# HybridRobotics/ilqr-iterative-tasks

Hardware: AMD Instinct MI355X
Metric: batched iLQR iterations/s (n=6,m=2,N=20) (higher is better)
Workload: dtype f64

## Files before the change

ilqr_iterative_tasks_amd/csrc/i2lqr_column_launch.hpp:

```cpp
#pragma once
#include <hip/hip_runtime.h>

#include "i2lqr_column_plan.hpp"
#include "i2lqr_devcfg.hpp"
#include "i2lqr_group.h"
#include "i2lqr_handle.hpp"
#include "i2lqr_host.hpp"
#include "i2lqr_kernels.h"
#include "i2lqr_wave_opt.h"

namespace i2lqr {

inline thread_local i2lqr_handle::Epilogue* t_epi = nullptr;

inline int64_t registered_ws(const i2lqr_handle* h) { return h->ws ? h->ws_bytes : -1; }
inline ColumnChoice column_kernel(const i2lqr_handle* h, int64_t B, bool early_exit) {
  return column_kernel(h->geo, h->fit, h->col, h->model.form(), registered_ws(h), B, early_exit);
}

inline int wave_lds_check(const i2lqr_handle* h, bool chained) {
  const size_t need = wave_lds_need(h->fit, h->model, chained);
  if (need <= h->geo.max_dyn_lds) return I2LQR_OK;
  const WaveForm f = h->model.form(chained);
  const int n_obs = h->model.records();
  char with[64];
  if (f == WAVE_OBS)
    snprintf(with, sizeof(with), "\"obstacles\" = %d", n_obs);
  else
    snprintf(with, sizeof(with), "%s and %d obstacle record%s",
             chained ? "\"wave_chain\"" : wave_phrase(f), n_obs, n_obs > 1 ? "s" : "");
  return fail(I2LQR_ERR_UNSUPPORTED, "horizon %d with %s needs %zu B of LDS per wavefront (> %zu KiB)",
              h->cfg.N, with, need, h->geo.max_dyn_lds / 1024);
}

template <class T, class Sys> struct Launch {
  static constexpr int n = Sys::n, m = Sys::m, LANES = 64;
  static constexpr bool kBicycle = m == 2 && n + m <= 8;
  using Cfg = DevCfg<T, n, m>;

  static unsigned grid(int64_t B) { return (unsigned)B; }

  static int prepare(i2lqr_handle* h) {
    h->lanes = LANES;
    h->fit.lds_wave = (size_t)Layout<Sys>(h->cfg.N).total * sizeof(T);
    h->fit.lds_wave_fstep = kWaveHasFstep<Sys> ? wave_fstep_lds_bytes<T, Sys>(h->cfg.N) : 0;
    const size_t lds = h->fit.lds_wave;
    if (lds > h->geo.max_dyn_lds)
      return fail(I2LQR_ERR_UNSUPPORTED, "horizon %d needs %zu B of LDS per wavefront (> %zu KiB)",
                  h->cfg.N, lds, h->geo.max_dyn_lds / 1024);
    if (lds > h->geo.default_dyn_lds)
      for (const void* kernel :
           {(const void*)k_iterate<T, Sys, LANES, false>, (const void*)k_iterate<T, Sys, LANES, true>,
            (const void*)k_backward<T, Sys, LANES, false>, (const void*)k_backward<T, Sys, LANES, true>,
            (const void*)k_forward<T, Sys, LANES, false>, (const void*)k_forward<T, Sys, LANES, true>,
            (const void*)k_rollout<T, Sys, LANES, false>, (const void*)k_rollout<T, Sys, LANES, true>})
        HIP_TRY(hipFuncSetAttribute(kernel, hipFuncAttributeMaxDynamicSharedMemorySize, (int)lds));
    return I2LQR_OK;
  }

  static int iterate(i2lqr_handle* h, const SolveIO& io, hipStream_t s) {
    const int64_t B = io.B;
    IterArgs<T> a = iter_args<T>(io);
    a.chains = h->col.opt_group_chains != 0;
#ifdef I2LQR_STAMPS
    a.dbg = (unsigned long long*)h->ws;
#endif
    const ColumnChoice choice = column_kernel(h, B, io.early_exit != 0);
    const ColumnKernel fk = choice.kernel;
    if (t_epi && (fk == K_GROUP || fk == K_GROUP16 || fk == K_GROUP_WS)) {
      a.qfun = t_epi->qfun;
      a.outer_iter = t_epi->outer_iter;
      a.max_relax_iter = t_epi->max_relax_iter;
      a.cost_it = (T*)t_epi->cost_it;
      if (t_epi->best_idx) {
        a.pick_part = (MinPair<T>*)t_epi->part;
        a.pick_ticket = h->ticket + h->ticket_next.fetch_add(1, std::memory_order_relaxed) %
                                        i2lqr_handle::kTickets;
        a.best_idx = t_epi->best_idx;
        a.best_cost = (T*)t_epi->best_cost;
      }
      t_epi->fused = true;
    }
#ifdef I2LQR_STAMPS
    constexpr bool stamps = true;
#else
    constexpr bool stamps = false;
#endif
    switch (fk) {
      case K_INVALID:
        return fail(I2LQR_ERR_UNSUPPORTED, "%s", choice.why);
      case K_SPEC:
      case K_SPEC16:
        if constexpr (kBicycle) {
          const int lanes = fk == K_SPEC16 ? 16 : 8;
          HIP_TRY(group_spec_iterate<T>(h->cfg, a, s, lanes,
                                        spec_wavefronts(h->geo, h->fit, lanes, B, false)));
          return I2LQR_OK;
        }
        break;
      case K_GROUP:
        if constexpr (kBicycle) {
          HIP_TRY(group_iterate<T>(h->cfg, a, s, stamps ? 1 : group8_wavefronts(h->geo, B)));
          return I2LQR_OK;
        }
        break;
      case K_GROUP16:
        if constexpr (kBicycle) {
          const int wavefronts =
              stamps ? 1 : group16_wavefronts(h->geo, B, h->col.opt_group_overlap != 0);
          HIP_TRY(group16_iterate<T>(h->cfg, a, s, wavefronts, !stamps && group16_fixed(h->fit, h->col)));
          return I2LQR_OK;
        }
        break;
      case K_GROUP_WS:
        if constexpr (kBicycle) {
          HIP_TRY(group_iterate_ws<T>(h->cfg, a, h->ws, s));
          return I2LQR_OK;
        }
        break;
      case K_QUAD:
        if constexpr (n + m == 16) {
          HIP_TRY(quad_iterate<T>(h->cfg, a, h->ws, s));
          return I2LQR_OK;
        }
        break;
      case K_WAVE_OPT:
        if (int rc = wave_lds_check(h, false)) return rc;
        HIP_TRY(wave_opt_launch<T>(h->cfg, a, h->model, false, h->fit.lds_wave, s));
        return I2LQR_OK;
      case K_WAVE:
        break;
    }
    const Cfg c = make_dev_cfg<T, n, m>(h->cfg);
    if constexpr (kWaveHasFstep<Sys>) {
      if (wave_fstep(h->geo, h->fit, h->col, B)) {
        with_weights(c.flags, [&](auto W) {
          hipLaunchKernelGGL((k_iterate<T, Sys, LANES, W, true>), dim3(grid(B)), dim3(64),
                             h->fit.lds_wave_fstep, s, c, a);
        });
        HIP_TRY(hipGetLastError());
        return I2LQR_OK;
      }
    }
    with_weights(c.flags, [&](auto W) {
      hipLaunchKernelGGL((k_iterate<T, Sys, LANES, W>), dim3(grid(B)), dim3(64), h->fit.lds_wave, s, c, a);
    });
    HIP_TRY(hipGetLastError());
    return I2LQR_OK;
  }
  static int names_pair(const i2lqr_handle*, int64_t, int) { return 0; }
  static int names_model(const i2lqr_handle*) { return 0; }
  static int solve_chained(i2lqr_handle* h, const SolveIO& io, int k, hipStream_t s) {
    const ChainPlan plan = chain_plan(h->geo, h->fit, h->col, h->model.form(), registered_ws(h), io.B);
    if (plan.kind == ChainPlan::REFUSED) return fail(I2LQR_ERR_UNSUPPORTED, "%s", plan.why);
    IterArgs<T> a = iter_args<T>(io);
    a.chain_len = k;
    a.chains = h->col.opt_group_chains != 0;
    if (plan.kind == ChainPlan::WAVE) {
      if (int rc = wave_lds_check(h, true)) return rc;
      HIP_TRY(wave_opt_launch<T>(h->cfg, a, h->model, true, h->fit.lds_wave, s));
    } else if constexpr (kBicycle) {
      HIP_TRY(group_spec_chain<T>(h->cfg, a, s));
    }
    return I2LQR_OK;
  }
  static int rollout(i2lqr_handle* h, int64_t B, void* X, void* U, const void* x_term, void* cost,
                     hipStream_t s) {
    const Cfg c = make_dev_cfg<T, n, m>(h->cfg);
    with_weights(c.flags, [&](auto W) {
      hipLaunchKernelGGL((k_rollout<T, Sys, LANES, W>), dim3(grid(B)), dim3(64), h->fit.lds_wave, s, c,
                         B, (T*)X, (T*)U, (const T*)x_term, (T*)cost);
    });
    HIP_TRY(hipGetLastError());
    return I2LQR_OK;
  }
  static int backward(i2lqr_handle* h, int64_t B, const void* X, const void* U, const void* x_term,
                      const void* lamb, const void* obs, void* K, void* k, hipStream_t s) {
    const Cfg c = make_dev_cfg<T, n, m>(h->cfg);
    with_weights(c.flags, [&](auto W) {
      hipLaunchKernelGGL((k_backward<T, Sys, LANES, W>), dim3(grid(B)), dim3(64), h->fit.lds_wave, s, c,
                         B, (const T*)X, (const T*)U, (const T*)x_term, (const T*)lamb,
                         (const T*)obs, (T*)K, (T*)k);
    });
    HIP_TRY(hipGetLastError());
    return I2LQR_OK;
  }
  static int forward(i2lqr_handle* h, int64_t B, const void* X, const void* U, const void* x_term,
                     const void* K, const void* k, void* Xn, void* Un, void* cost_new,
                     hipStream_t s) {
    const Cfg c = make_dev_cfg<T, n, m>(h->cfg);
    with_weights(c.flags, [&](auto W) {
      hipLaunchKernelGGL((k_forward<T, Sys, LANES, W>), dim3(grid(B)), dim3(64), h->fit.lds_wave, s, c,
                         B, (const T*)X, (const T*)U, (const T*)x_term, (const T*)K, (const T*)k,
                         (T*)Xn, (T*)Un, (T*)cost_new);
    });
    HIP_TRY(hipGetLastError());
    return I2LQR_OK;
  }
};

}
```

ilqr_iterative_tasks_amd/csrc/i2lqr_group.hpp:

```cpp
#pragma once
#include <hip/hip_runtime.h>
#include <stdint.h>

#include "i2lqr_systems.hpp"
#include "i2lqr_wave.hpp"

namespace i2lqr {

constexpr int kGroup = 8;
constexpr int kGroupsPerWave = 64 / kGroup;

template <class Sys> struct GroupPattern {
  static constexpr int n = Sys::n, m = Sys::m, W = n + m, NV = Sys::NVAR;
  static constexpr int dt_row(int b) {
    for (int i = 2; i < n; i++)
      if (i != b && Sys::pat(i, b) == 2) return i;
    return -1;
  }
  static constexpr bool column_ok(int b) {
    int extra = 0;
    for (int i = 0; i < n; i++) {
      const int code = Sys::pat(i, b);
      if (i < 2) {
        if (code == 2) return false;
        if (i == b && code != 1) return false;
        continue;
      }
      if (i == b) {
        if (code != 1) return false;
      } else if (code == 2) {
        extra++;
      } else if (code != 0) {
        return false;
      }
    }
    return extra <= 1;
  }
  static constexpr bool ok() {
    if (W > kGroup || n + 1 > kGroup || n < 2) return false;
    for (int b = 0; b < W; b++)
      if (!column_ok(b)) return false;
    return true;
  }
};

#ifndef I2LQR_GROUP_UNROLL
#define I2LQR_GROUP_UNROLL 4
#endif
template <class Sys, int G = kGroup> struct GLayout {
  static constexpr int n = Sys::n, m = Sys::m, W = n + m, NV = Sys::NVAR, NT = Sys::NTRIG;
  static constexpr int PW = 64 / G;
  static constexpr int KW = (n + 1 + 1) & ~1;
  static constexpr int R_JV = 0, R_ZERO = NV, R_ONE = NV + 1, R_LU = NV + 2, R_LUU = NV + 2 + m,
                       R_OB = NV + 2 + 2 * m, RW = (NV + 2 + 2 * m + 5 + 1) & ~1;
  int N;
  static constexpr int kT1Stride = 80;
  int XU0, XU1, Kk, R, TR0, TR1, total;
  __host__ __device__ explicit GLayout(int N_, bool ws = false) : N(N_) {
    int o = 0;
    XU0 = o; o += W * (N + 1); o = (o + 3) & ~3;
    XU1 = o; o += W * (N + 1); o = (o + 3) & ~3;
    Kk = o; o += ws ? m * KW : m * KW * N; o = (o + 3) & ~3;
    R = o; o += ws ? 0 : RW * (N + 1);
    TR0 = o; o += NT * (N + 1); o = (o + 3) & ~3;
    TR1 = o; o += NT * (N + 1); o = (o + 3) & ~3;
    o = (o + 3) & ~3;
    if (((o / 4) & 1) == 0) o += 4;
    total = o;
  }
  __host__ __device__ int t1_base() const { return PW * total; }
  __host__ __device__ int qt_base() const { return t1_base() + (G == kGroup ? PW * kT1Stride : 0); }
  __host__ __device__ int ctl_base() const { return (qt_base() + n * n + 3) & ~3; }
  __host__ __device__ int wave_words() const { return ctl_base() + 16; }
  __host__ __device__ int ws_rec() const { return 0; }
  __host__ __device__ int ws_gain() const { return RW * (N + 1); }
  __host__ __device__ int ws_words() const { return (RW * (N + 1) + m * KW * N + 15) & ~15; }
};


template <int L> __device__ __forceinline__ void bcast_fmac1(double& a, double s, double c) {
  asm("v_fmac_f64_dpp %0, %1, %2 row_newbcast:%3 row_mask:0xf bank_mask:0xf" : "+v"(a) : "v"(s), "v"(c), "n"(L));
}
template <int L> __device__ __forceinline__ void bcast_fmac1(float& a, float s, float c) {
  asm("v_fmac_f32_dpp %0, %1, %2 row_newbcast:%3 row_mask:0xf bank_mask:0xf" : "+v"(a) : "v"(s), "v"(c), "n"(L));
}
template <int L, class T, int R>
__device__ __forceinline__ void bcast_fmac(T (&a)[R], const T (&s)[R], T c) {
#pragma unroll
  for (int r = 0; r < R; r++) bcast_fmac1<L>(a[r], s[r], c);
}
template <int L> __device__ __forceinline__ double bcast_mov(double v) {
  long long x = __builtin_bit_cast(long long, v);
  x = __builtin_amdgcn_mov_dpp(x, 0x150 + L, 0xf, 0xf, false);
  return __builtin_bit_cast(double, x);
}
template <int L> __device__ __forceinline__ float bcast_mov(float v) {
  int x = __builtin_bit_cast(int, v);
  x = __builtin_amdgcn_mov_dpp(x, 0x150 + L, 0xf, 0xf, false);
  return __builtin_bit_cast(float, x);
}
template <class T, int R> __device__ __forceinline__ void dpp_ready(T (&v)[R]) {
  if constexpr (R == 8)
    asm("s_nop 1" : "+v"(v[0]), "+v"(v[1]), "+v"(v[2]), "+v"(v[3]), "+v"(v[4]), "+v"(v[5]), "+v"(v[6]), "+v"(v[7]));
  else if constexpr (R == 6)
    asm("s_nop 1" : "+v"(v[0]), "+v"(v[1]), "+v"(v[2]), "+v"(v[3]), "+v"(v[4]), "+v"(v[5]));
  else static_assert(R == 6 || R == 8, "dpp_ready: n + m of the bicycles");
}

template <class T, class Sys, bool WS = false, int G = kGroup, int NH = 0> struct GroupWorker {
  static constexpr int n = Sys::n, m = Sys::m, W = n + m, NV = Sys::NVAR, NT = Sys::NTRIG;
  static constexpr int NA = n + 1;
  using Cfg = DevCfg<T, n, m>;
  using GL = GLayout<Sys, G>;
  static_assert(G == kGroup || G == 16, "eight lanes per problem, or one 16-lane DPP row");
  static_assert(G == kGroup || !WS, "the workspace form is built for eight lanes per problem");
  static_assert(NH == 0 || (G == 16 && !WS), "the fixed-horizon form is the sixteen-lane LDS form");
  static __host__ __device__ constexpr int horizon(int cfg_N) { return NH > 0 ? NH : cfg_N; }
  using GP = GroupPattern<Sys>;
  static_assert(GP::ok(), "plant does not have the column structure this kernel is written for");
  const Cfg& c;
  const GL L;
  const Slice<T> S;
  const T* const Qt;
  const int g;
  const int N;
  __device__ __forceinline__ int loop_N() const {
    if constexpr (NH > 0) return c.N;
    else return N;
  }
  int oR, oKk;
  T* T1c;
  int rho;
  T* Wp = nullptr;

  int off_c0, off_c1;
  int off_l0, off_l1;
  int off_lu[m];
  T own, cdt;
  int rsrc;
#ifdef I2LQR_STAMPS
  mutable unsigned long long st_acc[8] = {0, 0, 0, 0, 0, 0, 0, 0}, st_t0 = 0, st_t1 = 0;
#endif

  __device__ GroupWorker(const Cfg& c_, T* smem, int lane)
      : GroupWorker(c_, smem + (lane / G) * GL(horizon(c_.N), WS).total,
                    smem + GL(horizon(c_.N), WS).qt_base(), lane % G,
                    GL(horizon(c_.N), WS).total) {
    const int p = lane / G;
    if constexpr (G == kGroup) T1c = smem + L.t1_base() + p * GL::kT1Stride;
    rho = (p >> 1) & 1;
  }
  __device__ __forceinline__ T* rec(int t) const {
    if constexpr (WS) return Wp + L.ws_rec() + t * GL::RW;
    else return S + oR + t * GL::RW;
  }
  __device__ __forceinline__ T* gain(int t) const {
    if constexpr (WS) return Wp + L.ws_gain() + t * (m * GL::KW);
    else return S + oKk + t * (m * GL::KW);
  }
  __device__ __forceinline__ T* gain_x(int t) const {
    if constexpr (WS) return S + oKk;
    else return S + oKk + t * (m * GL::KW);
  }
  __device__ __forceinline__ void ws_publish() const {
    if constexpr (WS) {
      __builtin_amdgcn_fence(__ATOMIC_RELEASE, "workgroup");
      __builtin_amdgcn_s_waitcnt(0);
      wave_sync();
      __builtin_amdgcn_fence(__ATOMIC_ACQUIRE, "workgroup");
    }
  }
  __device__ __forceinline__ int t1_word(int col, int row) const {
    return (row >> 1) * (2 * kGroup) + ((col + rho) & (kGroup - 1)) * 2 + (row & 1);
  }

  __device__ GroupWorker(const Cfg& c_, T* slice, const T* qt, int g_, int slice_words)
      : c(c_), L(horizon(c_.N), WS), S(make_slice(slice, slice_words, c_.trap, TAG_GROUP_LDS)),
        Qt(qt), g(g_), N(horizon(c_.N)) {
    oR = L.R; oKk = L.Kk;
    T1c = nullptr;
    rho = 0;
    off_c0 = GL::R_ZERO; off_c1 = GL::R_ZERO; off_l0 = GL::R_ZERO; off_l1 = GL::R_ZERO;
#pragma unroll
    for (int a = 0; a < m; a++) off_lu[a] = GL::R_ZERO;
    own = T(0); cdt = T(0); rsrc = 0;
    static_for_i<0, W>([&](auto b_) {
      constexpr int b = decltype(b_)::value;
      if (g == b && b < n) {
        constexpr int c0 = Sys::pat(0, b), c1 = Sys::pat(1, b);
        off_c0 = c0 == 0 ? GL::R_ZERO : (c0 == 1 ? GL::R_ONE : GL::R_JV + (c0 - 3));
        off_c1 = c1 == 0 ? GL::R_ZERO : (c1 == 1 ? GL::R_ONE : GL::R_JV + (c1 - 3));
        own = (b >= 2) ? T(1) : T(0);
        constexpr int r = GP::dt_row(b);
        cdt = r >= 0 ? c.dt : T(0);
        rsrc = r >= 0 ? r : 0;
        if (b < 2) {
          off_l0 = GL::R_OB + 2 + b;
          off_l1 = GL::R_OB + 3 + b;
        }
      }
    });
    if (g == n) {
      own = T(1);
      off_l0 = GL::R_OB + 0;
      off_l1 = GL::R_OB + 1;
#pragma unroll
      for (int a = 0; a < m; a++) off_lu[a] = GL::R_LU + a;
    }
    if constexpr (G == 16) {
      own = T(1);
      if (g == 0) off_c0 = GL::R_ZERO;
      if (g == 1) off_c1 = GL::R_ZERO;
    }
  }

  __device__ __forceinline__ T terminal_cost(const T (&x)[n], const T (&xT)[n]) const {
    T d[n];
#pragma unroll
    for (int i = 0; i < n; i++) d[i] = x[i] - xT[i];
    T acc = T(0);
#pragma unroll
    for (int j = 0; j < n; j++) {
      T col = T(0);
#pragma unroll
      for (int i = 0; i < n; i++) col += d[i] * Qt[i * n + j];
      acc += col * d[j];
    }
    return acc;
  }

  template <int i, int a> __device__ __forceinline__ void f_acc(T& acc, bool& first, T v,
                                                                const T (&jv)[NV]) const {
    constexpr int code = Sys::pat(i, a);
    if constexpr (code == 0) {
      return;
    } else if constexpr (code == 1) {
      acc = first ? v : acc + v;
      first = false;
    } else {
      const T f = code == 2 ? c.dt : jv[code >= 3 ? code - 3 : 0];
      acc = first ? f * v : t_fma(f, v, acc);
      first = false;
    }
  }

  __device__ __forceinline__ T rollout(int XUo, int TRo, const T (&xT)[n], bool chains) const {
    if constexpr (G == 16 && Sys::kTrigFreeTail) {
      if (__builtin_expect(chains, 1)) return rollout_row(XUo, TRo, xT);
    }
    T x[n], u[m], xn[n], tr[NT];
#pragma unroll
    for (int i = 0; i < n; i++) x[i] = S[XUo + i];
    const int N = loop_N();
    for (int t = 0; t < N; t++) {
#pragma unroll
      for (int a = 0; a < m; a++) u[a] = clip(S[XUo + t * W + n + a], -c.u_max[a], c.u_max[a]);
#pragma unroll
      for (int a = 0; a < m; a++) S[XUo + t * W + n + a] = u[a];
      Sys::trig(x, tr);
#pragma unroll
      for (int q = 0; q < NT; q++) S[TRo + t * NT + q] = tr[q];
      Sys::step_tr(c, x, u, tr, xn);
#pragma unroll
      for (int i = 0; i < n; i++) S[XUo + (t + 1) * W + i] = xn[i];
#pragma unroll
      for (int i = 0; i < n; i++) x[i] = xn[i];
    }
    Sys::trig(x, tr);
#pragma unroll
    for (int q = 0; q < NT; q++) S[TRo + N * NT + q] = tr[q];
    const T cost = terminal_cost(x, xT);
    wave_sync();
    return cost;
  }

  __device__ __forceinline__ T rollout_row(int XUo, int TRo, const T (&xT)[n]) const {
    static_assert(G == 16 && Sys::kTrigFreeTail, "see Sys::kTrigFreeTail");
    const int N = loop_N();
    for (int t = g; t < N; t += G) {
      T u[m];
#pragma unroll
      for (int a = 0; a < m; a++) u[a] = clip(S[XUo + t * W + n + a], -c.u_max[a], c.u_max[a]);
#pragma unroll
      for (int a = 0; a < m; a++) S[XUo + t * W + n + a] = u[a];
    }
    wave_sync();
    T x[n], u[m], xn[n], tr[NT];
#pragma unroll
    for (int i = 0; i < n; i++) x[i] = S[XUo + i];
#pragma unroll
    for (int q = 0; q < NT; q++) tr[q] = T(0);
    for (int t = 0; t < N; t++) {
#pragma unroll
      for (int a = 0; a < m; a++) u[a] = S[XUo + t * W + n + a];
      Sys::step_tr(c, x, u, tr, xn);
#pragma unroll
      for (int i = 2; i < n; i++) S[XUo + (t + 1) * W + i] = xn[i];
#pragma unroll
      for (int i = 2; i < n; i++) x[i] = xn[i];
    }
    const int rounds = (N + G) / G;
    for (int r = 0; r < rounds; r++) {
      const int t0 = g + r * G;
      const int t = t0 < N ? t0 : N;
      T xe[n];
      xe[0] = T(0); xe[1] = T(0);
#pragma unroll
      for (int i = 2; i < n; i++) xe[i] = S[XUo + t * W + i];
      Sys::trig(xe, tr);
#pragma unroll
      for (int q = 0; q < NT; q++) S[TRo + t * NT + q] = tr[q];
    }
    wave_sync();
    T un[m], trn[NT];
#pragma unroll
    for (int i = 0; i < n; i++) x[i] = S[XUo + i];
#pragma unroll
    for (int a = 0; a < m; a++) u[a] = S[XUo + n + a];
#pragma unroll
    for (int q = 0; q < NT; q++) tr[q] = S[TRo + q];
    for (int t = 0; t < N; t++) {
#pragma unroll
      for (int a = 0; a < m; a++) un[a] = S[XUo + (t + 1) * W + n + a];
#pragma unroll
      for (int q = 0; q < NT; q++) trn[q] = S[TRo + (t + 1) * NT + q];
      Sys::step_tr(c, x, u, tr, xn);
#pragma unroll
      for (int i = 0; i < n; i++) S[XUo + (t + 1) * W + i] = xn[i];
#pragma unroll
      for (int i = 0; i < n; i++) x[i] = xn[i];
#pragma unroll
      for (int a = 0; a < m; a++) u[a] = un[a];
#pragma unroll
      for (int q = 0; q < NT; q++) tr[q] = trn[q];
    }
    const T cost = terminal_cost(x, xT);
    wave_sync();
    return cost;
  }

  __device__ __forceinline__ void prep(int XUo, int TRo, const T (&ob)[6], T pa, T pb, int first,
                                       int stride, bool chains) const {
    if (__builtin_expect(chains, 1)) {
      if (sizeof(T) == 8 && __builtin_expect(c.fast_barrier, 1))
        prep_chains<true>(XUo, TRo, ob, pa, pb, first, stride);
      else
        prep_chains<false>(XUo, TRo, ob, pa, pb, first, stride);
    } else {
      prep_serial(XUo, TRo, ob, pa, pb, first, stride);
    }
    wave_sync();
    ws_publish();
  }

  template <bool FASTB>
  __device__ __forceinline__ void prep_chains(int XUo, int TRo, const T (&ob)[6], T pa, T pb,
                                              int first, int stride) const {
    static_assert(m == 2, "two inputs");
    const bool has_ob = ob[5] >= T(0);
    const int opt = has_ob ? (int)ob[5] : 0;
    const T spd_y = opt == 1 ? ob[4] : T(0), spd_x = opt == 2 ? ob[4] : T(0);
    const int rounds = (N + stride) / stride;
    for (int r = 0; r < rounds; r++) {
      const int t0 = first + r * stride;
      const int t = t0 < N ? t0 : N;
      const int ts = t0 < N ? t0 : N - 1;
      T* Rs = rec(ts);
      T* R = rec(t);
      if constexpr (FASTB) asm volatile("; record, short input barrier" ::: "memory");
      else asm volatile("; record, general input barrier" ::: "memory");
      T xe[n], tr[NT], u[m], jv[NV];
#pragma unroll
      for (int i = 0; i < n; i++) xe[i] = S[XUo + (ts + 1) * W + i];
#pragma unroll
      for (int a = 0; a < m; a++) u[a] = S[XUo + ts * W + n + a];
#pragma unroll
      for (int q = 0; q < NT; q++) tr[q] = S[TRo + (ts + 1) * NT + q];
      const T px = S[XUo + t * W + 0], py = S[XUo + t * W + 1];
      const T dz = opt == 2 ? px - (ob[0] - T(t) * spd_x) : px - ob[0];
      const T dy = opt == 1 ? py - (ob[1] + T(t) * spd_y) : py - ob[1];
      const T h = T(1) + c.safety_margin - (dz * pa * dz + dy * pb * dy);
      const T hd0 = T(-2) * pa * dz, hd1 = T(-2) * pb * dy;
      T e, e_hi[m], e_lo[m];
      if constexpr (FASTB) {
        const double xa[3] = {(double)(c.obs_q2 * h), (double)(c.ctrl_q2 * (u[0] - c.u_max[0])),
                              (double)(c.ctrl_q2 * (u[1] - c.u_max[1]))};
        double ea[3], rc[2];
        t_exp_d<false, 3, 2, true>(xa, ea);
        t_rcp2(ea[1], ea[2], &rc[0], &rc[1]);
        e = (T)ea[0];
#pragma unroll
        for (int a = 0; a < m; a++) {
          e_hi[a] = (T)ea[1 + a];
          e_lo[a] = c.ctrl_c[a] * (T)rc[a];
        }
      } else if constexpr (sizeof(T) == 8) {
        const double xa[5] = {(double)(c.obs_q2 * h), (double)(c.ctrl_q2 * (u[0] - c.u_max[0])),
                              (double)(c.ctrl_q2 * (-c.u_max[0] - u[0])),
                              (double)(c.ctrl_q2 * (u[1] - c.u_max[1])),
                              (double)(c.ctrl_q2 * (-c.u_max[1] - u[1]))};
        double ea[5];
        t_exp_d<false, 5, 0, true>(xa, ea);
        e = (T)ea[0];
// ... 108 lines not shown
#pragma unroll
        for (int r = 0; r < n; r++) {
          const T q = T(2) * Qt[i * n + r];
          vxx = (g == r) ? q : vxx;
          vx += q * dx[r];
        }
        va[i] = (g == n) ? vx : vxx;
      }
      va[0] += Rn[off_l0];
      va[1] += Rn[off_l1];
    }
    const int gcol = g < GL::KW ? g : GL::KW - 1;
    struct Rec { T jv[NV], luu[m], c0, c1, l0, l1, lrow[m]; };
    Rec ra, rb;
    auto load_record = [&](int t, Rec& r) __attribute__((always_inline)) {
      const T* R = rec(t);
#pragma unroll
      for (int q = 0; q < NV; q++) r.jv[q] = R[GL::R_JV + q];
#pragma unroll
      for (int a = 0; a < m; a++) r.luu[a] = R[GL::R_LUU + a];
      r.c0 = R[off_c0];
      r.c1 = R[off_c1];
      r.l0 = R[off_l0];
      r.l1 = R[off_l1];
#pragma unroll
      for (int a = 0; a < m; a++) r.lrow[a] = R[off_lu[a]];
    };
    load_record(N - 1, ra);
    auto step = [&](const int t, Rec& rc, Rec& rn) __attribute__((always_inline)) {
      if constexpr (WS) load_record(t > 0 ? t - 1 : 0, rn);
      const T (&jv)[NV] = rc.jv;
      const T (&luu)[m] = rc.luu;
      const T (&lrow)[m] = rc.lrow;
      const T c0 = rc.c0, c1 = rc.c1, l0 = rc.l0, l1 = rc.l1;
      STAMP_BEGIN();
      T t1[W];
      static_for_i<0, W>([&](auto a_) {
        constexpr int a = decltype(a_)::value;
        T acc = T(0);
        bool first = true;
        static_for_i<0, n>([&](auto i_) {
          constexpr int i = decltype(i_)::value;
          f_acc<i, a>(acc, first, va[i], jv);
        });
        t1[a] = acc;
      });
#pragma unroll
      for (int a = 0; a < W; a++) T1c[t1_word(g, a)] = t1[a];
      wave_sync();
      STAMP_END(1);
      T h[W];
      {
        T s0[W], s1[W], sr[W];
#pragma unroll
        for (int a = 0; a < W; a++) {
          s0[a] = T1c[t1_word(0, a)];
          s1[a] = T1c[t1_word(1, a)];
          sr[a] = T1c[t1_word(rsrc, a)];
        }
#pragma unroll
        for (int a = 0; a < W; a++) {
          T acc = c0 * s0[a];
          acc = t_fma(c1, s1[a], acc);
          acc = t_fma(own, t1[a], acc);
          acc = t_fma(cdt, sr[a], acc);
          h[a] = acc;
        }
        h[0] += l0;
        h[1] += l1;
#pragma unroll
        for (int a = 0; a < m; a++) h[n + a] += lrow[a];
      }
      STAMP_END(2);
      T Quu[m * m], Qinv[m * m];
      static_for_i<0, m>([&](auto a_) {
        constexpr int a = decltype(a_)::value;
        static_for_i<0, m>([&](auto b_) {
          constexpr int b = decltype(b_)::value;
          T acc = T(0);
          bool first = true;
          static_for_i<0, n>([&](auto i_) {
            constexpr int i = decltype(i_)::value;
            if constexpr (Sys::pat(i, n + b) != 0) f_acc<i, n + b>(acc, first, T1c[t1_word(i, n + a)], jv);
          });
          Quu[a * m + b] = (a == b ? luu[a] : T(0)) + acc;
        });
      });
      if constexpr (GENERAL) quu_inverse(Quu, lamb, Qinv);
      else t_quu_inverse2_pd(Quu, lamb, Qinv, &bad);
      STAMP_END(3);
      T kc[m];
#pragma unroll
      for (int a = 0; a < m; a++) {
        T acc = T(0);
#pragma unroll
        for (int b = 0; b < m; b++) acc = t_fma(Qinv[a * m + b], h[n + b], acc);
        kc[a] = -acc;
      }
      T* Kt = gain_x(t);
      if constexpr (WS) {
        T* Kg = gain(t);
#pragma unroll
        for (int a = 0; a < m; a++) {
          Kt[a * GL::KW + gcol] = kc[a];
          if (commit) Kg[a * GL::KW + gcol] = kc[a];
        }
      } else {
#pragma unroll
        for (int a = 0; a < m; a++)
          if (commit) Kt[a * GL::KW + gcol] = kc[a];
      }
      wave_sync();
      STAMP_END(4);
      T kr[m][n];
#pragma unroll
      for (int a = 0; a < m; a++)
#pragma unroll
        for (int i = 0; i < n; i++) kr[a][i] = Kt[a * GL::KW + i];
      if constexpr (!WS) load_record(t > 0 ? t - 1 : 0, rn);
      T qk[m];
#pragma unroll
      for (int a = 0; a < m; a++) {
        T acc = T(0);
#pragma unroll
        for (int b = 0; b < m; b++) acc = t_fma(Quu[a * m + b], kc[b], acc);
        qk[a] = acc;
      }
#pragma unroll
      for (int i = 0; i < n; i++) {
        T acc = T(0);
#pragma unroll
        for (int a = 0; a < m; a++) acc = t_fma(kr[a][i], qk[a], acc);
        va[i] = h[i] - acc;
      }
      STAMP_END(5);
    };
    int t = N - 1;
    if constexpr (I2LQR_GROUP_UNROLL >= 4) {
      for (; t >= 3; t -= 4) {
        step(t, ra, rb);
        step(t - 1, rb, ra);
        step(t - 2, ra, rb);
        step(t - 3, rb, ra);
      }
    }
    for (; t >= 1; t -= 2) {
      step(t, ra, rb);
      step(t - 1, rb, ra);
    }
    if (t == 0) step(0, ra, rb);
    ws_publish();
    return bad;
  }

  template <bool GENERAL>
  __device__ __forceinline__ bool backward_row(int XUo, const T (&xT)[n], T lamb, bool commit) const {
    T vb[n];
    terminal_base(XUo, xT, vb);
    return backward_row_from<GENERAL>(vb, lamb, commit);
  }
  __device__ __forceinline__ void terminal_base(int XUo, const T (&xT)[n], T (&vb)[n]) const {
    T dx[n];
#pragma unroll
    for (int i = 0; i < n; i++) dx[i] = S[XUo + N * W + i] - xT[i];
    const int gq = g < n ? g : 0;
#pragma unroll
    for (int i = 0; i < n; i++) {
      T vx = T(0);
#pragma unroll
      for (int r = 0; r < n; r++) vx += (T(2) * Qt[i * n + r]) * dx[r];
      const T vxx = T(2) * Qt[i * n + gq];
      vb[i] = (g == n) ? vx : (g < n ? vxx : T(0));
    }
  }
  template <bool GENERAL>
  __device__ __forceinline__ bool backward_row_from(const T (&vb)[n], T lamb, bool commit) const {
    static_assert(GL::KW > n + 1, "the padding word of a gain row takes the stores of idle lanes");
    bool bad = false;
    T va[n];
    {
      const T* Rn = rec(N);
#pragma unroll
      for (int i = 0; i < n; i++) va[i] = vb[i];
      va[0] += Rn[off_l0];
      va[1] += Rn[off_l1];
    }
    const int gcol = (commit && g <= n) ? g : GL::KW - 1;
    T cdr[n];
#pragma unroll
    for (int r = 0; r < n; r++) cdr[r] = (rsrc == r) ? cdt : T(0);
    struct Rec { T jv[NV], luu[m], c0, c1, l0, l1, lrow[m]; };
    Rec ra, rb;
    constexpr bool FIXED = NH > 0 && !GENERAL;
    const T* const R0 = rec(0);
    const T *pc0 = R0, *pc1 = R0, *pl0 = R0, *pl1 = R0, *plu[m];
#pragma unroll
    for (int a = 0; a < m; a++) plu[a] = R0;
    if constexpr (FIXED) {
      pc0 = R0 + off_c0; pc1 = R0 + off_c1; pl0 = R0 + off_l0; pl1 = R0 + off_l1;
#pragma unroll
      for (int a = 0; a < m; a++) plu[a] = R0 + off_lu[a];
    }
    auto load_record = [&](int t, Rec& r) __attribute__((always_inline)) {
      if constexpr (FIXED) {
        const int o = t * GL::RW;
#pragma unroll
        for (int q = 0; q < NV; q++) r.jv[q] = R0[o + GL::R_JV + q];
#pragma unroll
        for (int a = 0; a < m; a++) r.luu[a] = R0[o + GL::R_LUU + a];
        r.c0 = pc0[o];
        r.c1 = pc1[o];
        r.l0 = pl0[o];
        r.l1 = pl1[o];
#pragma unroll
        for (int a = 0; a < m; a++) r.lrow[a] = plu[a][o];
      } else {
        const T* R = rec(t);
#pragma unroll
        for (int q = 0; q < NV; q++) r.jv[q] = R[GL::R_JV + q];
#pragma unroll
        for (int a = 0; a < m; a++) r.luu[a] = R[GL::R_LUU + a];
        r.c0 = R[off_c0];
        r.c1 = R[off_c1];
        r.l0 = R[off_l0];
        r.l1 = R[off_l1];
#pragma unroll
        for (int a = 0; a < m; a++) r.lrow[a] = R[off_lu[a]];
      }
    };
    auto f_entry = [&](auto k_, auto b_, const T (&jv)[NV]) __attribute__((always_inline)) {
      constexpr int code = Sys::pat(decltype(k_)::value, n + decltype(b_)::value);
      if constexpr (code == 1) return T(1);
      else if constexpr (code == 2) return c.dt;
      else return jv[code >= 3 ? code - 3 : 0];
    };
    load_record(N - 1, ra);
    auto step = [&](const int t, Rec& rc, Rec& rn) __attribute__((always_inline)) {
      const T (&jv)[NV] = rc.jv;
      T t1[W];
      static_for_i<0, W>([&](auto a_) {
        constexpr int a = decltype(a_)::value;
        T acc = T(0);
        bool first = true;
        static_for_i<0, n>([&](auto i_) {
          constexpr int i = decltype(i_)::value;
          f_acc<i, a>(acc, first, va[i], jv);
        });
        t1[a] = acc;
      });
      dpp_ready(t1);
      load_record(t > 0 ? t - 1 : 0, rn);
      T Quu[m * m], Qinv[m * m];
      {
        T t1u[m];
#pragma unroll
        for (int a = 0; a < m; a++) t1u[a] = t1[n + a];
        static_for_i<0, m>([&](auto b_) {
          constexpr int b = decltype(b_)::value;
          T col[m];
#pragma unroll
          for (int a = 0; a < m; a++) col[a] = (a == b) ? rc.luu[a] : T(0);
          static_for_i<0, n>([&](auto k_) {
            constexpr int k = decltype(k_)::value;
            if constexpr (Sys::pat(k, n + b) != 0) bcast_fmac<k>(col, t1u, f_entry(k_, b_, jv));
          });
#pragma unroll
          for (int a = 0; a < m; a++) Quu[a * m + b] = col[a];
        });
      }
      auto h_rows = [&](auto r0_, auto& hr) __attribute__((always_inline)) {
        constexpr int r0 = decltype(r0_)::value;
        constexpr int R = sizeof(hr) / sizeof(T);
        T src[R];
#pragma unroll
        for (int a = 0; a < R; a++) { src[a] = t1[r0 + a]; hr[a] = t1[r0 + a]; }
        bcast_fmac<0>(hr, src, rc.c0);
        bcast_fmac<1>(hr, src, rc.c1);
        static_for_i<2, n>([&](auto r_) {
          constexpr int r = decltype(r_)::value;
          constexpr bool used = [] {
            for (int b = 0; b < n; b++)
              if (GP::dt_row(b) == r) return true;
            return false;
          }();
          if constexpr (used) bcast_fmac<r>(hr, src, cdr[r]);
        });
      };
      T hu[m], hx[n];
      h_rows(std::integral_constant<int, n>{}, hu);
#pragma unroll
      for (int a = 0; a < m; a++) hu[a] += rc.lrow[a];
      if constexpr (GENERAL) quu_inverse(Quu, lamb, Qinv);
      else t_quu_inverse2_pd(Quu, lamb, Qinv, &bad);
      h_rows(std::integral_constant<int, 0>{}, hx);
      hx[0] += rc.l0;
      hx[1] += rc.l1;
      T pk[m], kc[m];
#pragma unroll
      for (int a = 0; a < m; a++) {
        T acc = T(0);
#pragma unroll
        for (int b = 0; b < m; b++) acc = t_fma(Qinv[a * m + b], hu[b], acc);
        pk[a] = acc;
        kc[a] = -acc;
      }
      T* Kt = gain_x(t);
#pragma unroll
      for (int a = 0; a < m; a++) Kt[a * GL::KW + gcol] = kc[a];
      T qk[m];
#pragma unroll
      for (int a = 0; a < m; a++) {
        T acc = T(0);
#pragma unroll
        for (int b = 0; b < m; b++) acc = t_fma(Quu[a * m + b], kc[b], acc);
        qk[a] = acc;
      }
      T vn[n];
#pragma unroll
      for (int i = 0; i < n; i++) vn[i] = hx[i];
      static_for_i<0, n>([&](auto i_) {
        constexpr int i = decltype(i_)::value;
#pragma unroll
        for (int a = 0; a < m; a++) bcast_fmac1<i>(vn[i], pk[a], qk[a]);
      });
#pragma unroll
      for (int i = 0; i < n; i++) va[i] = vn[i];
    };
    STAMP_BEGIN();
    if constexpr (FIXED) {
      static_for_i<0, NH>([&](auto i_) {
        constexpr int i = decltype(i_)::value;
        if constexpr (i % 2 == 0) step(NH - 1 - i, ra, rb);
        else step(NH - 1 - i, rb, ra);
      });
    } else {
      int t = loop_N() - 1;
      if constexpr (I2LQR_GROUP_UNROLL >= 4) {
        for (; t >= 3; t -= 4) {
          step(t, ra, rb);
          step(t - 1, rb, ra);
          step(t - 2, ra, rb);
          step(t - 3, rb, ra);
        }
      }
      for (; t >= 1; t -= 2) {
        step(t, ra, rb);
        step(t - 1, rb, ra);
      }
      if (t == 0) step(0, ra, rb);
    }
    STAMP_END(1);
    wave_sync();
    return bad;
  }

  __device__ __forceinline__ T forward_row(int XUo, int XUn, int TRn, const T (&xT)[n],
                                           bool* bad, bool chains, int TRo) const {
    static_assert(G == 16 && m == 2, "two inputs on the two halves of a 16-lane row");
    const int half = g >> 3;
    const T umax = half ? c.u_max[1] : c.u_max[0];
    T x[n], u[m], xn[n], tr[NT];
#pragma unroll
    for (int i = 0; i < n; i++) x[i] = S[XUo + i];
#pragma unroll
    for (int i = 0; i < n; i++) S[XUn + i] = x[i];
#ifdef I2LQR_FORWARD_X0_TRIG
    chains = false;
#endif
    if (__builtin_expect(chains, 1)) {
#pragma unroll
      for (int q = 0; q < NT; q++) tr[q] = S[TRo + q];
    } else {
      Sys::template trig_g<false>(x, tr, bad);
    }
#pragma unroll
    for (int q = 0; q < NT; q++) S[TRn + q] = tr[q];
    static_assert(!WS, "gain rows and records are neighbours in the LDS slice");
    auto pXo = S + XUo;
    auto pXn = S + XUn;
    auto pG = S + (oKk + half * GL::KW);
    auto pTR = S + (TRn + half * NT);
    T xo[n], uo, kk[NA];
    auto load_step = [&](auto k_) __attribute__((always_inline)) {
      constexpr int k = decltype(k_)::value;
#pragma unroll
      for (int j = 0; j < n; j++) xo[j] = pXo[k * W + j];
      uo = pXo[k * W + n + half];
#pragma unroll
      for (int j = 0; j < NA; j++) kk[j] = pG[k * (m * GL::KW) + j];
    };
    load_step(std::integral_constant<int, 0>{});
    auto step = [&](auto k_, const T (&trc)[NT]) __attribute__((always_inline)) {
      constexpr int k = decltype(k_)::value;
      T acc = T(0);
#pragma unroll
      for (int j = 0; j < n; j++) acc = t_fma(kk[j], x[j] - xo[j], acc);
      const T ua = clip(uo + kk[n] + acc, -umax, umax);
      load_step(std::integral_constant<int, k + 1>{});
      pXn[k * W + n + half] = ua;
      u[0] = bcast_mov<0>(ua);
      u[1] = bcast_mov<8>(ua);
      Sys::step_tr(c, x, u, trc, xn);
#pragma unroll
      for (int i = 0; i < n; i++) pXn[(k + 1) * W + i] = xn[i];
#pragma unroll
      for (int i = 0; i < n; i++) x[i] = xn[i];
    };
#define I2LQR_FORWARD_ROW_PAIR()                                                                   \
    {                                                                                              \
      step(std::integral_constant<int, 0>{}, tr);                                 \
      T sc[NT], tr1[NT];                                                                           \
      Sys::trig_heading_fast(half ? Sys::next_heading(c, x) : Sys::heading(x), sc, bad);           \
      _Pragma("unroll") for (int q = 0; q < NT; q++) pTR[NT + q] = sc[q];  \
      _Pragma("unroll") for (int q = 0; q < NT; q++) {                                             \
        tr1[q] = bcast_mov<0>(sc[q]);                                                              \
        tr[q] = bcast_mov<8>(sc[q]);                   \
      }                                                                                            \
      step(std::integral_constant<int, 1>{}, tr1);                                \
      pXo = pXo + 2 * W;                                                                           \
      pXn = pXn + 2 * W;                                                                           \
      pG = pG + 2 * (m * GL::KW);                                                                  \
      pTR = pTR + 2 * NT;                                                                          \
    }
#define I2LQR_FORWARD_ROW_LAST()                     \
    {                                                                                              \
      step(std::integral_constant<int, 0>{}, tr);                                                  \
      Sys::template trig_g<false>(x, tr, bad);                                                     \
      _Pragma("unroll") for (int q = 0; q < NT; q++) S[TRn + N * NT + q] = tr[q];                  \
    }
    if constexpr (NH > 0) {
      static_for_i<0, NH / 2>([&](auto) __attribute__((always_inline)) I2LQR_FORWARD_ROW_PAIR());
      if constexpr (NH % 2 != 0) I2LQR_FORWARD_ROW_LAST()
    } else {
      int t = 0;
      for (; t + 1 < N; t += 2) I2LQR_FORWARD_ROW_PAIR()
      if (t < N) I2LQR_FORWARD_ROW_LAST()
    }
#undef I2LQR_FORWARD_ROW_PAIR
#undef I2LQR_FORWARD_ROW_LAST
    const T cost = terminal_cost(x, xT);
    wave_sync();
    return cost;
  }

  template <bool GENERAL>
  __device__ __forceinline__ T forward(int XUo, int XUn, int TRn, const T (&xT)[n],
                                       bool* bad, bool chains = false, int TRo = 0) const {
    if constexpr (G == 16 && !GENERAL && Sys::kHeadingAhead && m == 2)
      return forward_row(XUo, XUn, TRn, xT, bad, chains, TRo);
    const int N = loop_N();
    T x[n], u[m], xn[n], tr[NT];
#pragma unroll
    for (int i = 0; i < n; i++) x[i] = S[XUo + i];
#pragma unroll
    for (int i = 0; i < n; i++) S[XUn + i] = x[i];
    T xo[n], uo[m];
    struct Gains { T kk[m][NA]; };
    Gains ga, gb;
    auto load_gains = [&](int t, Gains& q) __attribute__((always_inline)) {
      const T* Kg = gain(t);
#pragma unroll
      for (int a = 0; a < m; a++)
#pragma unroll
        for (int j = 0; j < NA; j++) q.kk[a][j] = Kg[a * GL::KW + j];
    };
    auto load_step = [&](int t, Gains& q) __attribute__((always_inline)) {
#pragma unroll
      for (int j = 0; j < n; j++) xo[j] = S[XUo + t * W + j];
#pragma unroll
      for (int a = 0; a < m; a++) uo[a] = S[XUo + t * W + n + a];
      if constexpr (!WS) load_gains(t, q);
    };
    if constexpr (WS) {
      load_gains(0, ga);
      load_gains(N >= 2 ? 1 : 0, gb);
    }
    load_step(0, ga);
    auto step = [&](const int t, Gains& q, Gains& qn) __attribute__((always_inline)) {
#pragma unroll
      for (int a = 0; a < m; a++) {
        T acc = T(0);
#pragma unroll
        for (int j = 0; j < n; j++) acc = t_fma(q.kk[a][j], x[j] - xo[j], acc);
        u[a] = clip(uo[a] + q.kk[a][n] + acc, -c.u_max[a], c.u_max[a]);
      }
      if constexpr (WS) {
        load_gains(t + 2 < N ? t + 2 : N - 1, q);
        load_step(t + 1 < N ? t + 1 : t, qn);
      } else {
        load_step(t + 1 < N ? t + 1 : t, q);
      }
#pragma unroll
      for (int a = 0; a < m; a++) S[XUn + t * W + n + a] = u[a];
      Sys::template trig_g<GENERAL>(x, tr, bad);
#pragma unroll
      for (int q = 0; q < NT; q++) S[TRn + t * NT + q] = tr[q];
      Sys::step_tr(c, x, u, tr, xn);
#pragma unroll
      for (int i = 0; i < n; i++) S[XUn + (t + 1) * W + i] = xn[i];
#pragma unroll
      for (int i = 0; i < n; i++) x[i] = xn[i];
    };
    int t = 0;
    if constexpr (WS) {
      for (; t + 1 < N; t += 2) {
        step(t, ga, gb);
        step(t + 1, gb, ga);
      }
      if (t < N) step(t, ga, gb);
    } else {
      if constexpr (I2LQR_GROUP_UNROLL >= 4) {
        for (; t + 3 < N; t += 4) {
          step(t, ga, ga);
          step(t + 1, ga, ga);
          step(t + 2, ga, ga);
          step(t + 3, ga, ga);
        }
      }
      for (; t + 1 < N; t += 2) {
        step(t, ga, ga);
        step(t + 1, ga, ga);
      }
      if (t < N) step(t, ga, ga);
    }
    Sys::template trig_g<GENERAL>(x, tr, bad);
#pragma unroll
    for (int q = 0; q < NT; q++) S[TRn + N * NT + q] = tr[q];
    const T cost = terminal_cost(x, xT);
    wave_sync();
    return cost;
  }
};

__device__ __forceinline__ int idx_div(int e, int d, float rcp_d) {
  int q = (int)((float)e * rcp_d);
  const int r = e - q * d;
  q += (r >= d) ? 1 : 0;
  q -= (r < 0) ? 1 : 0;
  return q;
}

template <class T, class Sys, int H, bool WS, int G, int NH>
__device__ __forceinline__ void group_iterate_body(const DevCfg<T, Sys::n, Sys::m>& c,
                                                   const IterArgs<T>& a, T* ws) {
  static_assert(!(WS && H > 1), "the workspace form runs without helper wavefronts");
  constexpr int n = Sys::n, m = Sys::m, W = n + m;
#ifdef I2LQR_STAMPS
  constexpr bool OVL = false;
#else
  constexpr bool OVL = G == 16 && H >= 3;
#endif
  using GL = GLayout<Sys, G>;
  extern __shared__ __align__(16) unsigned char gsmem_raw[];
  T* smem = reinterpret_cast<T*>(gsmem_raw);
  const int lane = threadIdx.x & 63, hv = threadIdx.x >> 6;
#ifdef I2LQR_STAMPS
  unsigned long long st_k0, st_k1, st_k2, st_k3;
  asm volatile("s_memtime %0\n\ts_waitcnt lgkmcnt(0)" : "=s"(st_k0)::"memory");
#endif
  const int64_t prob0 = (int64_t)blockIdx.x * GL::PW + lane / G;
  const bool real = prob0 < a.B;
  const int64_t prob = real ? prob0 : a.B - 1;
  GroupWorker<T, Sys, WS, G, NH> w(c, smem, lane);
  const int N = NH > 0 ? NH : c.N, g = w.g;
  const float rN = 1.0f / (float)N, rN1 = 1.0f / (float)(N + 1), rnN = 1.0f / (float)(n * N);
  const GL& L = w.L;
  const auto S = w.S;
  if constexpr (WS) w.Wp = ws + prob0 * (int64_t)L.ws_words();

  if (H == 1 || hv == 0) {
    const T* gX = a.X + prob * (int64_t)(n * (N + 1));
    if (g < n) S[L.XU0 + g] = gX[g * (N + 1)];
    const T* gU = a.U + prob * (int64_t)(m * N);
    for (int e = g; e < m * N; e += G) {
      const int aa = idx_div(e, N, rN), t = e - aa * N;
      S[L.XU0 + t * W + n + aa] = gU[e];
    }
    for (int e = lane; e < n * n; e += 64) smem[L.qt_base() + e] = c.Qt[e];
  }
  T xT[n], ob[6];
#pragma unroll
  for (int i = 0; i < n; i++) xT[i] = a.x_term[prob * n + i];
#pragma unroll
  for (int q = 0; q < 6; q++) ob[q] = a.obs ? a.obs[prob * 6 + q] : T(q == 5 ? -1 : 1);
  T lamb = a.lamb[prob];
  wave_sync();

  int cur = 0;
  const T ob_pa = T(1) / (ob[2] * ob[2]), ob_pb = T(1) / (ob[3] * ob[3]);
  int* const ctl = reinterpret_cast<int*>(smem + L.ctl_base());
  if constexpr (H > 1) {
    if (hv > 0) {
      const int h0 = OVL ? hv - 1 : hv, hs = OVL ? H - 1 : H;
      for (;;) {
        __syncthreads();
        const int flags = ctl[8];
        if (!(flags & 1)) break;
        if (flags & 2) {
          const int pc = ctl[lane / G];
          w.prep(pc ? L.XU1 : L.XU0, pc ? L.TR1 : L.TR0, ob, ob_pa, ob_pb, h0 * G + g, hs * G,
                 a.chains != 0);
        }
        __syncthreads();
      }
      if constexpr (OVL) {
        if (real && a.K) {
          T* const gK = a.K + prob * (int64_t)(m * n * N);
          T* const gk = a.k + prob * (int64_t)(m * N);
          for (int t = h0 * G + g; t < N; t += hs * G) {
            const T* Kt = w.gain(t);
            T kv[m][n + 1];
#pragma unroll
            for (int aa = 0; aa < m; aa++)
#pragma unroll
              for (int j = 0; j <= n; j++) kv[aa][j] = Kt[aa * GL::KW + j];
#pragma unroll
            for (int aa = 0; aa < m; aa++) {
#pragma unroll
              for (int j = 0; j < n; j++) gK[(aa * n + j) * N + t] = kv[aa][j];
              gk[aa * N + t] = kv[aa][n];
            }
          }
        }
      }
      return;
    }
  }
  T vb[n];
#pragma unroll
  for (int i = 0; i < n; i++) vb[i] = T(0);
  const bool chains = a.chains != 0;
  T cost = w.rollout(L.XU0, L.TR0, xT, chains);
  int it = 0, status = a.early_exit ? 2  : 0 ;
  T cost_ret = cost;
  bool fresh = true, active = a.n_iters > 0;
#ifdef I2LQR_STAMPS
  asm volatile("s_memtime %0\n\ts_waitcnt lgkmcnt(0)" : "=s"(st_k1)::"memory");
#endif
  while (__any(active)) {
    const int XUo = cur ? L.XU1 : L.XU0, XUn = cur ? L.XU0 : L.XU1;
    const int TRo = cur ? L.TR1 : L.TR0, TRn = cur ? L.TR0 : L.TR1;
#ifdef I2LQR_STAMPS
    {
      auto& st_t0 = w.st_t0; auto& st_t1 = w.st_t1; auto& st_acc = w.st_acc;
      STAMP_BEGIN();
      if (__any(fresh)) w.prep(XUo, TRo, ob, ob_pa, ob_pb, g, G, chains);
      STAMP_END(0);
    }
#else
    if constexpr (H > 1) {
      const bool do_prep = __any(fresh);
      if (g == 0) ctl[lane / G] = cur;
      if (lane == 0) ctl[8] = 1 | (do_prep ? 2 : 0);
      __syncthreads();
      if constexpr (OVL) {
        if (do_prep) w.terminal_base(XUo, xT, vb);
      } else {
        if (do_prep) w.prep(XUo, TRo, ob, ob_pa, ob_pb, g, H * G, chains);
      }
      __syncthreads();
    } else {
      if (__any(fresh)) w.prep(XUo, TRo, ob, ob_pa, ob_pb, g, G, chains);
    }
#endif
    if constexpr (OVL) {
      if (__builtin_expect(__any(w.template backward_row_from<false>(vb, lamb, active)), 0))
        w.template backward_row_from<true>(vb, lamb, active);
    } else {
      if (__builtin_expect(__any(w.template backward<false>(XUo, xT, lamb, active)), 0))
        w.template backward<true>(XUo, xT, lamb, active);
    }
    T cost_new;
    {
#ifdef I2LQR_STAMPS
      auto& st_t0 = w.st_t0; auto& st_t1 = w.st_t1; auto& st_acc = w.st_acc;
      STAMP_BEGIN();
#endif
      bool big = false;
      cost_new = w.template forward<false>(XUo, XUn, TRn, xT, &big, chains, TRo);
      if (__builtin_expect(__any(big), 0)) cost_new = w.template forward<true>(XUo, XUn, TRn, xT, &big);
#ifdef I2LQR_STAMPS
      STAMP_END(6);
#endif
    }
    {
      const bool acc = active && cost_new < cost, rej = active && !(cost_new < cost);
      const T lamb_dn = lamb / c.lamb_factor, lamb_up = lamb * c.lamb_factor;
      const bool conv = t_abs((cost_new - cost) / cost) < c.eps;
      it += active ? 1 : 0;
      fresh = acc;
      cur ^= acc ? 1 : 0;
      lamb = acc ? lamb_dn : (rej ? lamb_up : lamb);
      cost_ret = acc ? cost_new : (rej ? cost : cost_ret);
      cost = acc ? cost_new : cost;
      const bool stop_conv = acc && conv, stop_lamb = rej && lamb > c.max_lamb;
      const int ended = stop_conv ? 1 : 3;
      if (a.early_exit) {
        status = (stop_conv || stop_lamb) ? ended : status;
        active = active && !(stop_conv || stop_lamb);
      } else {
        status = (status == 0 && (stop_conv || stop_lamb)) ? ended : status;
      }
      active = active && it < a.n_iters;
    }
  }
#ifdef I2LQR_STAMPS
  asm volatile("s_memtime %0\n\ts_waitcnt lgkmcnt(0)" : "=s"(st_k2)::"memory");
#endif
  if constexpr (H > 1) {
    if (lane == 0) ctl[8] = 0;
    __syncthreads();
  }
  if (!t_isfinite(cost_ret)) status = 4;

  if (OVL && real) {
    const int XUo = cur ? L.XU1 : L.XU0;
    T* const gX = a.X + prob * (int64_t)(n * (N + 1));
    T* const gU = a.U + prob * (int64_t)(m * N);
    for (int t = g; t <= N; t += G) {
      T xu[W];
#pragma unroll
      for (int i = 0; i < W; i++) xu[i] = S[XUo + t * W + i];
#pragma unroll
      for (int i = 0; i < n; i++) gX[i * (N + 1) + t] = xu[i];
      if (t < N) {
#pragma unroll
        for (int aa = 0; aa < m; aa++) gU[aa * N + t] = xu[n + aa];
      }
    }
    if (g == 0) {
      a.lamb[prob] = lamb;
      a.cost[prob] = cost_ret;
      if (a.iters) a.iters[prob] = it;
      if (a.status) a.status[prob] = status;
    }
  }
  if (!OVL && real) {
    const int XUo = cur ? L.XU1 : L.XU0;
    T* gX = a.X + prob * (int64_t)(n * (N + 1));
    for (int e = g; e < n * (N + 1); e += G) {
      const int i = idx_div(e, N + 1, rN1), t = e - i * (N + 1);
      gX[e] = S[XUo + t * W + i];
// ... 302 lines not shown
```

Measured before the change: 83.73 million.

## Software-pipeline fixed-horizon forward rollout loads and use asm negate in fixed path

Adds a fixed-horizon forward_row_ahead path that prefetches the next step's nominal state, input and gains from LDS into double-buffered registers while the current step computes, with sched barriers to keep the loads early. It also changes the gain negation in the fixed backward path to an inline-asm 64-bit integer add of the sign bit, and enables the fixed group16 variant even when timing stamps are compiled in. The prefetching is meant to hide LDS latency in the serial forward pass, at the cost of more live registers and possible occupancy loss.

Result: faster. 85.04 million (median of 6 runs) (+1.6%).

```diff
diff --git a/ilqr_iterative_tasks_amd/csrc/i2lqr_column_launch.hpp b/ilqr_iterative_tasks_amd/csrc/i2lqr_column_launch.hpp
--- a/ilqr_iterative_tasks_amd/csrc/i2lqr_column_launch.hpp
+++ b/ilqr_iterative_tasks_amd/csrc/i2lqr_column_launch.hpp
@@ -108,7 +108,7 @@
         if constexpr (kBicycle) {
           const int wavefronts =
               stamps ? 1 : group16_wavefronts(h->geo, B, h->col.opt_group_overlap != 0);
-          HIP_TRY(group16_iterate<T>(h->cfg, a, s, wavefronts, !stamps && group16_fixed(h->fit, h->col)));
+          HIP_TRY(group16_iterate<T>(h->cfg, a, s, wavefronts, group16_fixed(h->fit, h->col)));
           return I2LQR_OK;
         }
         break;
diff --git a/ilqr_iterative_tasks_amd/csrc/i2lqr_group.hpp b/ilqr_iterative_tasks_amd/csrc/i2lqr_group.hpp
--- a/ilqr_iterative_tasks_amd/csrc/i2lqr_group.hpp
+++ b/ilqr_iterative_tasks_amd/csrc/i2lqr_group.hpp
@@ -99,6 +99,12 @@
   x = __builtin_amdgcn_mov_dpp(x, 0x150 + L, 0xf, 0xf, false);
   return __builtin_bit_cast(float, x);
 }
+__device__ __forceinline__ double neg_one_op(double x) {
+  double d;
+  asm("v_lshl_add_u64 %0, %1, 0, %2" : "=v"(d) : "v"(x), "s"(0x8000000000000000ull));
+  return d;
+}
+__device__ __forceinline__ float neg_one_op(float x) { return -x; }
 template <class T, int R> __device__ __forceinline__ void dpp_ready(T (&v)[R]) {
   if constexpr (R == 8)
     asm("s_nop 1" : "+v"(v[0]), "+v"(v[1]), "+v"(v[2]), "+v"(v[3]), "+v"(v[4]), "+v"(v[5]), "+v"(v[6]), "+v"(v[7]));
@@ -813,7 +819,8 @@
 #pragma unroll
         for (int b = 0; b < m; b++) acc = t_fma(Qinv[a * m + b], hu[b], acc);
         pk[a] = acc;
-        kc[a] = -acc;
+        if constexpr (FIXED) kc[a] = neg_one_op(acc);
+        else kc[a] = -acc;
       }
       T* Kt = gain_x(t);
 #pragma unroll
@@ -868,6 +875,7 @@
   __device__ __forceinline__ T forward_row(int XUo, int XUn, int TRn, const T (&xT)[n],
                                            bool* bad, bool chains, int TRo) const {
     static_assert(G == 16 && m == 2, "two inputs on the two halves of a 16-lane row");
+    if constexpr (NH > 0) return forward_row_ahead(XUo, XUn, TRn, xT, bad, chains, TRo);
     const int half = g >> 3;
     const T umax = half ? c.u_max[1] : c.u_max[0];
     T x[n], u[m], xn[n], tr[NT];
@@ -939,16 +947,99 @@
       Sys::template trig_g<false>(x, tr, bad);                                                     \
       _Pragma("unroll") for (int q = 0; q < NT; q++) S[TRn + N * NT + q] = tr[q];                  \
     }
-    if constexpr (NH > 0) {
-      static_for_i<0, NH / 2>([&](auto) __attribute__((always_inline)) I2LQR_FORWARD_ROW_PAIR());
-      if constexpr (NH % 2 != 0) I2LQR_FORWARD_ROW_LAST()
-    } else {
+    {
       int t = 0;
       for (; t + 1 < N; t += 2) I2LQR_FORWARD_ROW_PAIR()
       if (t < N) I2LQR_FORWARD_ROW_LAST()
     }
 #undef I2LQR_FORWARD_ROW_PAIR
 #undef I2LQR_FORWARD_ROW_LAST
+    const T cost = terminal_cost(x, xT);
+    wave_sync();
+    return cost;
+  }
+
+  __device__ __forceinline__ T forward_row_ahead(int XUo, int XUn, int TRn, const T (&xT)[n],
+                                                 bool* bad, bool chains, int TRo) const {
+    static_assert(NH > 0 && G == 16 && m == 2 && !WS, "forward_row's form, fixed horizon");
+    const int half = g >> 3;
+    const T umax = half ? c.u_max[1] : c.u_max[0];
+    const auto pXo = S + XUo;
+    const auto pXn = S + XUn;
+    const auto pG = S + (oKk + half * GL::KW);
+    const auto pTR = S + (TRn + half * NT);
+    struct In { T xo[n], uo, kk[NA]; };
+    In sa, sb;
+    auto load_step = [&](auto t_, In& s) __attribute__((always_inline)) {
+      constexpr int t = decltype(t_)::value;
+#pragma unroll
+      for (int j = 0; j < n; j++) s.xo[j] = pXo[t * W + j];
+      s.uo = pXo[t * W + n + half];
+#pragma unroll
+      for (int j = 0; j < NA; j++) s.kk[j] = pG[t * (m * GL::KW) + j];
+    };
+    load_step(std::integral_constant<int, 0>{}, sa);
+    __builtin_amdgcn_sched_barrier(0);
+    T x[n], u[m], xn[n], tr[NT];
+#pragma unroll
+    for (int i = 0; i < n; i++) x[i] = S[XUo + i];
+#pragma unroll
+    for (int i = 0; i < n; i++) S[XUn + i] = x[i];
+#ifdef I2LQR_FORWARD_X0_TRIG
+    chains = false;
+#endif
+    if (__builtin_expect(chains, 1)) {
+#pragma unroll
+      for (int q = 0; q < NT; q++) tr[q] = S[TRo + q];
+    } else {
+      Sys::template trig_g<false>(x, tr, bad);
+    }
+#pragma unroll
+    for (int q = 0; q < NT; q++) S[TRn + q] = tr[q];
+    auto step = [&](auto t_, const In& sc, In& sn, const T (&trc)[NT], auto&& later)
+        __attribute__((always_inline)) {
+      constexpr int t = decltype(t_)::value;
+      load_step(std::integral_constant<int, t + 1>{}, sn);
+      if constexpr (t % 2 == 0) __builtin_amdgcn_sched_barrier(0);
+      T acc = T(0);
+#pragma unroll
+      for (int j = 0; j < n; j++) acc = t_fma(sc.kk[j], x[j] - sc.xo[j], acc);
+      const T ua = clip(sc.uo + sc.kk[n] + acc, -umax, umax);
+      u[0] = bcast_mov<0>(ua);
+      u[1] = bcast_mov<8>(ua);
+      if constexpr (t > 0) {
+#pragma unroll
+        for (int i = 0; i < n; i++) pXn[t * W + i] = x[i];
+      }
+      pXn[t * W + n + half] = ua;
+      later();
+      Sys::step_tr(c, x, u, trc, xn);
+#pragma unroll
+      for (int i = 0; i < n; i++) x[i] = xn[i];
+    };
+    static_for_i<0, NH / 2>([&](auto p_) __attribute__((always_inline)) {
+      constexpr int t = 2 * decltype(p_)::value;
+      step(std::integral_constant<int, t>{}, sa, sb, tr, [] {});
+      T sc[NT], tr1[NT];
+      Sys::trig_heading_fast(half ? Sys::next_heading(c, x) : Sys::heading(x), sc, bad);
+#pragma unroll
+      for (int q = 0; q < NT; q++) {
+        tr1[q] = bcast_mov<0>(sc[q]);
+        tr[q] = bcast_mov<8>(sc[q]);
+      }
+      step(std::integral_constant<int, t + 1>{}, sb, sa, tr1, [&]() __attribute__((always_inline)) {
+#pragma unroll
+        for (int q = 0; q < NT; q++) pTR[(t + 1) * NT + q] = sc[q];
+      });
+    });
+    if constexpr (NH % 2 != 0) {
+      step(std::integral_constant<int, NH - 1>{}, sa, sb, tr, [] {});
+      Sys::template trig_g<false>(x, tr, bad);
+#pragma unroll
+      for (int q = 0; q < NT; q++) S[TRn + NH * NT + q] = tr[q];
+    }
+#pragma unroll
+    for (int i = 0; i < n; i++) pXn[NH * W + i] = x[i];
     const T cost = terminal_cost(x, xT);
     wave_sync();
     return cost;
```
